# bark-simulator/planner-miqp

Measured on AMD Instinct MI355X. Metric: MIQP solves/sec to 1% gap, 2-agent x 20-step x 32-region, higher is better.
Workload: dtype f64

## Files before the change

planner_miqp_amd/csrc/kernels.hip:

```cpp
#include <hip/hip_runtime.h>

#include "host_inst.hpp"

#ifndef MIQP_RHO
#define MIQP_RHO 1.0e5
#endif

#ifndef MIQP_IPM_WPE
#define MIQP_IPM_WPE 3
#endif

#ifdef MIQP_ABLATE
#define MIQP_ABL (B.abl)
#else
#define MIQP_ABL 0
#endif
namespace miqp {

constexpr double RHO_EL = MIQP_RHO;
constexpr double FEAS_TOL = 1.0e-6;
constexpr double QP_TOL = 1.0e-6;
#ifndef MIQP_T0
#define MIQP_T0 1.0e-3
#endif
// ... 1936 lines not shown
    const double thr = B.far_cap > 0 && !B.inst_mode[inst] ? B.near_thr[inst] : 1e300;
    int nk = 0, nfar = 0, nnear = 0; double fmin_ = 1e300;
    for (int a = 0; a < nalt; ++a) {
      const double cb = objlb + clift[a];
      if (inc_now < 1e300 && (inc_now - cb) <= gapi * (1e-10 + fabs(inc_now))) { if (B.stats) atomicAdd(&B.stats[56], 1ull); continue; }
      int negm = 0;
      if (chosen.kind == 3 && ck[a] >= 0 && ck[a] < N && (B.seq_kinds & 0x10000) == 0) {
        negm = 1 << (int)comp[base + ck[a] * stride];
        for (int a2 = 1; a2 < a; ++a2) if (ck[a2] == ck[a]) negm |= 1 << ca[a2];
      }
      const bool tf = (cb - cst) > thr && B.batch_depth[node] != REPAIR_ROOT;
      k_ck[nk] = ck[a]; k_ca[nk] = ca[a]; k_neg[nk] = negm; k_ord[nk] = a; k_bnd[nk] = cb - cst;
      k_pos[nk] = tf ? (0x40000000 | nfar++) : nnear++;
      if (tf) fmin_ = fmin(fmin_, cb - cst);
      nk++;
    }
    int fbase = 0, obase = 0, ob2 = 0, extra2 = 0; bool okalloc = true;
    if (nnear > 0) {
      obase = atomicAdd(&B.open_count[inst], nnear);
      if (obase + nnear > B.open_cap) {
        for (int q = obase; q < obase + nnear && q < B.open_cap; ++q) { size_t oi = ((size_t)B.open_sel * B.n_slots + slot) * B.open_cap + q; B.open_bound[oi] = 1e300; B.open_node[oi] = -1; B.open_depth[oi] = 0; }
        if (B.far_cap > 0) { for (int q = 0; q < nk; ++q) if (!(k_pos[q] & 0x40000000)) { k_pos[q] = 0x40000000 | nfar++; fmin_ = fmin(fmin_, k_bnd[q]); } }
        else okalloc = false;
        nnear = 0; obase = 0;
      }
    }
    const int nnear_kept = nnear;
    if (nfar > 0) {
      fbase = atomicAdd(&B.far_count[inst], nfar);
      if (fbase + nfar <= B.far_cap) atomicMin(&B.far_minkey[inst], d2key(fmin_));
      else {
        for (int q = fbase; q < fbase + nfar && q < B.far_cap; ++q) { B.far_bound[(size_t)slot * B.far_cap + q] = 1e300; B.far_node[(size_t)slot * B.far_cap + q] = -1; }
        int extra = 0;
        for (int q = 0; q < nk; ++q) if (k_pos[q] & 0x40000000) k_pos[q] = 0x20000000 | extra++;
        nfar = 0;
        ob2 = atomicAdd(&B.open_count[inst], extra); extra2 = extra;
        if (ob2 + extra > B.open_cap) {
          okalloc = false;
          for (int q = ob2; q < ob2 + extra && q < B.open_cap; ++q) { size_t oi = ((size_t)B.open_sel * B.n_slots + slot) * B.open_cap + q; B.open_bound[oi] = 1e300; B.open_node[oi] = -1; B.open_depth[oi] = 0; }
        }
        sh_base[3] = ob2;
      }
    }
    if (okalloc && nk > 0) {
      unsigned int h = atomicAdd(B.free_head, (unsigned int)nk);
      if ((int)(*B.free_limit - h) >= nk) {
        for (int q = 0; q < nk; ++q) slots[q] = B.free_q[(h + q) % (unsigned int)B.pool_cap];
      } else {
        int nb = atomicAdd(B.pool_count, nk);
        if (nb + nk > B.pool_cap) okalloc = false;
        for (int q = 0; q < nk; ++q) slots[q] = nb + q;
      }
    }
    if (!okalloc) {
      atomicOr(&B.inst_flags[inst], 1);
      for (int q = fbase; q < fbase + nfar; ++q) { B.far_bound[(size_t)slot * B.far_cap + q] = 1e300; B.far_node[(size_t)slot * B.far_cap + q] = -1; }
      for (int q = obase; q < obase + nnear_kept && q < B.open_cap; ++q) { size_t oi = ((size_t)B.open_sel * B.n_slots + slot) * B.open_cap + q; B.open_bound[oi] = 1e300; B.open_node[oi] = -1; B.open_depth[oi] = 0; }
      for (int q = ob2; q < ob2 + extra2 && q < B.open_cap; ++q) { size_t oi = ((size_t)B.open_sel * B.n_slots + slot) * B.open_cap + q; B.open_bound[oi] = 1e300; B.open_node[oi] = -1; B.open_depth[oi] = 0; }
      nk = 0;
    }
    if (B.stats && nk > 0) { atomicAdd(&B.stats[43], 1ull); atomicAdd(&B.stats[44], (unsigned long long)nk); atomicAdd(&B.stats[48 + chosen.kind], 1ull); atomicAdd(&B.stats[52 + chosen.kind], (unsigned long long)nk); }
    sh_base[0] = fbase; sh_base[1] = obase; sh_base[2] = nk;
  }
  __syncthreads();
  PROF_T(te5);
  const int nk = sh_base[2];
  if (nk <= 0) { FREE_NODE(); return; }
  {
    for (int q = 0; q < nk; ++q) {
      signed char* dst = B.pool_fix + (size_t)slots[q] * Y.fixlen;
      const int kk = k_ck[q]; const signed char av = (signed char)k_ca[q];
      int negidx = -1; const int negm = k_neg[q];
      if (chosen.kind == 3 && kk >= 0 && kk < N && (B.seq_kinds & 0x10000) == 0) negidx = Y.f_c2n + (chosen.c * N + kk) * 4 + chosen.o;
      if (kk != -2) {
        for (int k8 = lane; k8 < Y.fixlen / 8; k8 += 64) ((unsigned long long*)cfix)[k8] = ((const unsigned long long*)fix)[k8];
        __syncthreads();
        for (int j = jlo + lane; j <= jhi; j += 64) { const int k = base + j * stride; if (fix[k] < 0) { if (j < kk) cfix[k] = comp[k]; else if (j == kk) cfix[k] = av; } }
        __syncthreads();
        if (lane == 0 && negidx >= 0) cfix[negidx] = (signed char)negm;
        __syncthreads();
        for (int k8 = lane; k8 < Y.fixlen / 8; k8 += 64) ((unsigned long long*)dst)[k8] = ((const unsigned long long*)cfix)[k8];
        __syncthreads();
      } else
      for (int k = lane; k < Y.fixlen; k += 64) {
        signed char v = fix[k];
        int rel = k - base;
        if (v < 0 && rel >= 0 && rel % stride == 0) {
          int j = rel / stride;
          if (j >= jlo && j <= jhi) { if (j < kk) v = comp[k]; else if (j == kk) v = av; }
        }
        if (k == negidx) v = (signed char)negm;
        if (kk == -2) {
          v = (fix[k] < 0 && k < Y.f_c2n) ? comp[k] : fix[k];
          if ((B.opt2 & 0x10000) && fix[k] < 0 && k >= Y.f_env && k < Y.f_c2c && (k - Y.f_env) % 5 != 0) v = fix[k];
          if (B.probe_margin > 0.0 && fix[k] < 0 && ploose[k]) v = fix[k];
        }
        dst[k] = v;
      }
      if (B.pool_origin && lane == 0) {
        int cls = k_ord[q] > 0 ? 1 : 0;
        if (chosen.kind == 0 && cls) { const int rq = (int)comp[base + chosen.i * stride] >> 2, cq = k_ca[q] >> 2; const int dq = T[Y.i_regj + chosen.c * P + cq] - T[Y.i_regj + chosen.c * P + rq]; const int ad = abs(dq) % Y.R;
          cls = (k_ca[q] & 3) == 3 ? 3 : ((ad == 1 || ad == Y.R - 1) ? 1 : 2); }
        B.pool_origin[slots[q]] = (signed char)(kk == -2 ? 15 : 4 * chosen.kind + cls);
      }
    }
    if (B.pool_big && lane < nk) B.pool_big[slots[lane]] = pumped ? (unsigned char)((((big_parent >> 4) + 1) << 4) | 1) : (unsigned char)(big_parent & ~12);
    if (B.pool_Z) {
      for (int q = 0; q < nk; ++q) { if (slots[q] >= B.z_cap) continue; double* zd = B.pool_Z + (size_t)slots[q] * N * NZ; for (int k = lane; k < N * NZ; k += 64) zd[k] = Z[k]; }
    }
    if (B.pool_A) {
      const bool as_node = B.batch_A && B.batch_large && B.batch_large[node] <= 1;
      const unsigned short av_ = as_node ? B.batch_A[(size_t)node * 64 + lane] : (unsigned short)0xFFFFu;
      for (int q = 0; q < nk; ++q) { if (slots[q] >= B.z_cap) continue; B.pool_A[(size_t)slots[q] * 64 + lane] = av_; }
      if (B.ring_M && lane < nk && slots[lane] < B.z_cap) B.pool_Mtag[slots[lane]] = as_node ? B.batch_Mtag[node] : 0ull;
    }
    if (lane < nk) {
      int pd = B.batch_depth[node] >> 6;
      int pref = k_ord[lane];
      if (B.opt2 & 2) {
        pref = 0;
        for (int q = 0; q < nk; ++q) if (k_bnd[q] < k_bnd[lane] || (k_bnd[q] == k_bnd[lane] && q < lane)) pref++;
      }
      const int dw = k_ck[lane] == -2 ? (((pd + 2) << 6) | 63) : (((pd + 1) << 6) | (62 - (pref < 62 ? pref : 62)));
      if (k_pos[lane] & 0x40000000) {
        size_t oi = (size_t)slot * B.far_cap + sh_base[0] + (k_pos[lane] & 0x3FFFFFFF);
        B.far_bound[oi] = k_bnd[lane]; B.far_node[oi] = slots[lane]; B.far_depth[oi] = dw;
      } else {
        const int np_ = (k_pos[lane] & 0x20000000) ? sh_base[3] + (k_pos[lane] & 0x1FFFFFFF) : sh_base[1] + k_pos[lane];
        size_t oi = ((size_t)B.open_sel * B.n_slots + slot) * B.open_cap + np_;
        B.open_bound[oi] = k_bnd[lane]; B.open_node[oi] = slots[lane]; B.open_depth[oi] = dw;
      }
    }
  }
  FREE_NODE();
#ifdef MIQP_PROFILE
  { PROF_T(te6);
    if (lane == 0) { atomicAdd(&B.prof[100], (unsigned long long)(te1 - te0)); atomicAdd(&B.prof[101], (unsigned long long)(te2 - te1)); atomicAdd(&B.prof[102], (unsigned long long)(te3 - te2));
                     atomicAdd(&B.prof[103], (unsigned long long)(te4 - te3)); atomicAdd(&B.prof[104], (unsigned long long)(te5 - te4)); atomicAdd(&B.prof[105], (unsigned long long)(te6 - te5)); atomicAdd(&B.prof[106], 1ull); } }
#endif
#undef FREE_NODE
}

constexpr int SEL_THREADS = 1024;
constexpr int SEL_LOWSHIFT = 24;

__device__ inline int wave_append(int* counter, bool pred) {
  const unsigned long long mk = __ballot(pred);
  const int lane = threadIdx.x & 63;
  int base = 0;
  if (lane == (int)(__ffsll((long long)mk) - 1)) base = atomicAdd(counter, __popcll(mk));
  base = __shfl(base, mk ? (int)(__ffsll((long long)mk) - 1) : 0);
  return base + __popcll(mk & ((1ull << lane) - 1ull));
}

__global__ void __launch_bounds__(SEL_THREADS) select_kernel(DevBuf B, int round) {
  const Layout& Y = B.Y;
  const int slot = blockIdx.x, tid = threadIdx.x;
#ifdef MIQP_PROFILE
  if (slot == 0 && tid == 0) {
    const unsigned long long a = B.prof[120], b = B.prof[121], c = B.prof[122];
    if (b != 0 && a != ~0ull && a != 0) { B.prof[123] += b - a; B.prof[124] += b - c; B.prof[125] += 1; }
    B.prof[120] = ~0ull; B.prof[121] = 0; B.prof[122] = ~0ull;
  }
#endif
  const int inst = B.slot_inst[slot];
  if (inst < 0 || B.inst_done[inst] || B.inst_kill[inst]) { if (tid == 0) B.slot_demand[slot] = 0; }
  if (inst < 0) return;
  const int cap = B.open_cap;
  __shared__ int sh_take, sh_base, sh_m, sh_keep, sh_pick, sh_ties, sh_w, sh_mv, sh_all, sh_elig;
  __shared__ double sh_inc;
  __shared__ unsigned int hist[256], dhist[256], sh_wsum[4];
  __shared__ int sh_bin;
  __shared__ int sh_dkeep, sh_tiecnt, sh_ndef;
  __shared__ unsigned long long sh_thr2;
  __shared__ unsigned long long sh_prefix, sh_thr, sh_fmin;
  __shared__ double red[SEL_THREADS];
  if (B.inst_done[inst]) return;
  const size_t src = ((size_t)B.open_sel * B.n_slots + slot) * cap, dst = ((size_t)(1 - B.open_sel) * B.n_slots + slot) * cap;
  unsigned long long* keys = B.open_key + (size_t)slot * cap;
  PROF_T(ts0);
  if (tid == 0) {
    unsigned long long key = B.inc_key[inst];
    sh_inc = inc_from_key(key);
    sh_take = -1;
    sh_thr = key != B.inc_seen[inst] ? key : ~0ull;
    sh_fmin = ~0ull;
    sh_m = 0; sh_keep = 0; sh_pick = 0; sh_ties = 0; sh_ndef = 0;
  }
  __syncthreads();
  if (sh_thr != ~0ull) {
    const unsigned long long key = sh_thr;
    const int pbc = B.prev_bc < B.batch_cap ? B.prev_bc : B.batch_cap;
    for (int k = tid; k < pbc; k += SEL_THREADS) if (B.batch_candkey[k] == key && B.batch_candinst[k] == inst) atomicMin(&sh_fmin, d2key(B.batch_obj[k]));
    __syncthreads();
    const unsigned long long bo = sh_fmin;
    if (tid == 0) sh_dkeep = 0x7FFFFFFF;
    __syncthreads();
    if (bo != ~0ull) for (int k = tid; k < pbc; k += SEL_THREADS) if (B.batch_candkey[k] == key && B.batch_candinst[k] == inst && d2key(B.batch_obj[k]) == bo) atomicMin(&sh_dkeep, k);
    __syncthreads();
    if (tid == 0 && sh_dkeep != 0x7FFFFFFF) { sh_take = sh_dkeep; B.inc_seen[inst] = key; }
  }
  __syncthreads();
  if (sh_take >= 0) {
    const int bslot = sh_take;
    const signed char* cf = B.batch_comp + (size_t)bslot * Y.fixlen; signed char* df = B.inc_fix + (size_t)inst * Y.fixlen;
    for (int k = tid; k < Y.fixlen; k += SEL_THREADS) df[k] = cf[k];
    const double* zs = B.batch_Z + (size_t)bslot * Y.N * Y.nz; double* zd = B.inc_Z + (size_t)inst * Y.N * Y.nz;
    for (int k = tid; k < Y.N * Y.nz; k += SEL_THREADS) zd[k] = zs[k];
    if (B.inc_A && B.batch_A && B.batch_Mtag) {
      if (tid < 64) B.inc_A[(size_t)inst * 64 + tid] = B.batch_A[(size_t)bslot * 64 + tid];
      if (tid == 0) B.inc_Mtag[inst] = B.batch_Mtag[bslot];
    }
    if (tid == 0) { B.inc_obj[inst] = B.batch_obj[bslot]; if (B.inst_lns) B.inst_lns[inst] |= 1; }
  }
  __syncthreads();
  if (B.inst_kill[inst]) {
    int nn = B.open_count[inst]; if (nn > cap) nn = cap;
    for (int k = tid; k < nn; k += SEL_THREADS) { const int nd = B.open_node[src + k]; if (nd >= 0) { unsigned int q_ = atomicAdd(B.free_tail, 1u); B.free_q[q_ % (unsigned int)B.pool_cap] = nd; } }
    int fn = B.far_cap > 0 ? B.far_count[inst] : 0; if (fn > B.far_cap) fn = B.far_cap;
    for (int k = tid; k < fn; k += SEL_THREADS) { const int nd = B.far_node[(size_t)slot * (size_t)B.far_cap + k]; if (nd >= 0) { unsigned int q_ = atomicAdd(B.free_tail, 1u); B.free_q[q_ % (unsigned int)B.pool_cap] = nd; } }
    __syncthreads();
    if (tid == 0) {
      B.open_count[inst] = 0; if (B.far_cap > 0) B.far_count[inst] = 0;
      atomicOr(&B.inst_flags[inst], 2); B.inst_done[inst] = 1; atomicSub(B.active_insts, 1);
    }
    return;
  }
  PROF_T(ts1);
  const double inc = fmin(sh_inc < 1e300 ? B.inc_obj[inst] : 1e300, B.inc_ext[inst]);
  const double cst = B.inst_const[inst];
  const double gap = B.inst_gap[inst];
  int n = B.open_count[inst]; if (n > cap) n = cap;
  auto prunable = [&](double b) { return inc < 1e300 && (inc - (b + cst)) <= gap * (1e-10 + fabs(inc)); };
  auto radix = [&](auto keyf, int cnt, int need) -> int {
    if (tid == 0) { sh_prefix = 0ull; sh_all = 0; }
    __syncthreads();
    for (int shift = 56; shift >= SEL_LOWSHIFT; shift -= 8) {
      if (tid < 256) hist[tid] = 0u;
      __syncthreads();
      const unsigned long long prefix = sh_prefix;
      const unsigned long long himask = shift == 56 ? 0ull : (~0ull << (shift + 8));
      for (int k = tid; k < cnt; k += SEL_THREADS) {
        unsigned long long key = keyf(k);
        if (key != ~0ull && (key & himask) == prefix) atomicAdd(&hist[(key >> shift) & 255ull], 1u);
      }
      __syncthreads();
      if (tid == 0) sh_bin = 256;
      unsigned int hv = 0, hx = 0;
      if (tid < 256) {
        hv = hist[tid]; hx = hv;
#pragma unroll
        for (int o = 1; o < 64; o <<= 1) { const unsigned int y = __shfl_up(hx, o); if ((tid & 63) >= o) hx += y; }
        if ((tid & 63) == 63) sh_wsum[tid >> 6] = hx;
      }
      __syncthreads();
      if (tid < 256) {
#pragma unroll
        for (int w = 0; w < 3; ++w) if (w < (tid >> 6)) hx += sh_wsum[w];
        if (hx >= (unsigned int)need) atomicMin(&sh_bin, tid);
        if (tid == 255) sh_wsum[3] = hx;
      }
      __syncthreads();
      {
        const int bin0 = sh_bin;
        if (tid == (bin0 < 256 ? bin0 : 255)) {
          const int bin = bin0 < 256 ? bin0 : 255;
          const unsigned int cum = bin0 < 256 ? hx - hv : sh_wsum[3];
          if (bin0 >= 256 && shift == 56) sh_all = 1;
          sh_prefix = prefix | ((unsigned long long)bin << shift);
          sh_pick = need - (int)cum;
          sh_tiecnt = (int)hv;
        }
      }
      __syncthreads();
      need = sh_pick;
      if (sh_all) break;
    }
    __syncthreads();
    return need;
  };
  const unsigned long long lowmask = (1ull << SEL_LOWSHIFT) - 1ull;
  int keep = cap / 4; { const int k2 = 2 * B.batch_cap > 65536 ? 2 * B.batch_cap : 65536; if (keep > k2) keep = k2; }
  const int spill_at = 2 * keep;
  const size_t fb = (size_t)slot * (size_t)B.far_cap;
  int fc = B.far_cap > 0 ? B.far_count[inst] : 0; if (fc > B.far_cap) fc = B.far_cap;
  const int dive_every = (B.seq_kinds >> 18) & 3;
  const bool periodic = dive_every == 0 ? (round & 3) == 3 : (dive_every == 1 ? false : (dive_every == 2 ? (round & 7) == 7 : (round & 1) == 1));
  bool pool_tight;
  { const int pc = *B.pool_count; const long long live = (long long)(pc < B.pool_cap ? pc : B.pool_cap) - (long long)(int)(*B.free_tail - *B.free_head);
    pool_tight = live > (long long)B.pool_cap / 10 * 9; }
  const bool lists_full = B.far_cap > 0 ? fc > B.far_cap / 4 * 3 : n > cap / 2;
  const bool dive = !(inc < 1e300) || periodic || lists_full || pool_tight;
  auto order_key = [&](double b, int dp) -> unsigned long long {
    const int dbias = (B.seq_kinds >> 24) & 3;
    const double bb = dbias ? b - (dbias == 1 ? 1e-4 : (dbias == 2 ? 1e-3 : 1e-2)) * fabs(b) * (double)(dp >> 6) : b;
    if (dive) { const unsigned long long kd = ((unsigned long long)(0xFFFF - (dp < 0xFFFF ? dp : 0xFFFF)) << 48) | (d2key(fmax(b, -1e300)) >> 16); return kd == ~0ull ? ~0ull - 1 : kd; }
    const double kv = fmax(bb, -1e300);
    const unsigned long long key = d2key(kv); return key == ~0ull ? ~0ull - 1 : key;
  };
  PROF_T(ts2);
  for (int k = tid; k < 256; k += SEL_THREADS) dhist[k] = 0u;
  __syncthreads();
  double lb = 1e300; int mloc = 0, ndef = 0;
  const bool big_round = B.probe_every <= 1 || (round % B.probe_every) == B.probe_every - 1;
  for (int k = tid; k < n; k += SEL_THREADS) {
    double b = B.open_bound[src + k]; int nd = B.open_node[src + k]; int dp = B.open_depth[src + k];
    unsigned long long key = ~0ull;
    if (nd < 0) { keys[k] = key; continue; }
    if (prunable(b)) {
      unsigned int q_ = atomicAdd(B.free_tail, 1u); B.free_q[q_ % (unsigned int)B.pool_cap] = nd;
    } else {
      lb = fmin(lb, b);
      key = order_key(b, dp);
      if (!big_round && is_probe_word(dp)) { key = ~0ull - 1; ndef++; }
      atomicAdd(&dhist[(dp >> 6) > 255 ? 255 : (dp >> 6)], 1u);
      mloc++;
    }
    keys[k] = key;
  }
  if (mloc) atomicAdd(&sh_m, mloc);
  if (ndef) atomicAdd(&sh_ndef, ndef);
  __syncthreads();
  int m = sh_m;
  PROF_T(ts3);
  if (fc > 0 && m < keep / 4 && cap - n >= 64) {
    auto fkey = [&](int k) -> unsigned long long {
      const double b = B.far_bound[fb + k];
      if (B.far_node[fb + k] < 0 || prunable(b)) return ~0ull;
      const unsigned long long key = d2key(b); return key == ~0ull ? ~0ull - 1 : key;
    };
    int stride = fc > 4 * keep ? (fc + keep - 1) / keep : 1;
    if (stride > 1 && (fc + stride - 1) / stride > cap - n) stride = (fc + (cap - n) - 1) / (cap - n);
    if (stride > 1) {
      const int ns = (fc + stride - 1) / stride;
      for (int j = tid; j < ns; j += SEL_THREADS) keys[n + j] = fkey(j * stride);
      __syncthreads();
      int need_s = (keep - m) / stride; if (need_s < 1) need_s = 1;
      radix([&](int k) { return keys[n + k]; }, ns, need_s);
    } else radix(fkey, fc, keep - m);
    const unsigned long long thr = sh_all ? ~0ull : sh_prefix;
    if (tid == 0) { sh_w = 0; sh_mv = 0; sh_fmin = ~0ull; }
    __syncthreads();
    int room = cap - n; if (room > keep - m) room = keep - m; if (room < 0) room = 0;
    constexpr int PER = 4;
    for (int c0 = 0; c0 < fc; c0 += SEL_THREADS * PER) {
      double eb[PER]; int en[PER], ed[PER], act[PER];
#pragma unroll
      for (int j = 0; j < PER; ++j) {
        const int k = c0 + j * SEL_THREADS + tid;
        act[j] = -1;
        if (k < fc) {
          eb[j] = B.far_bound[fb + k]; en[j] = B.far_node[fb + k]; ed[j] = B.far_depth[fb + k];
          if (en[j] < 0) act[j] = -1;
          else if (prunable(eb[j])) act[j] = 0;
          else { unsigned long long key = d2key(eb[j]); if (key == ~0ull) key = ~0ull - 1; act[j] = ((key & ~lowmask) <= thr) ? 2 : 1; }
        }
      }
      __syncthreads();
#pragma unroll
      for (int j = 0; j < PER; ++j) {
        if (act[j] == 0) { unsigned int q_ = atomicAdd(B.free_tail, 1u); B.free_q[q_ % (unsigned int)B.pool_cap] = en[j]; }
        int t = wave_append(&sh_mv, act[j] == 2);
        if (act[j] == 2) {
          if (t < room) {
            B.open_bound[src + n + t] = eb[j]; B.open_node[src + n + t] = en[j]; B.open_depth[src + n + t] = ed[j]; keys[n + t] = order_key(eb[j], ed[j]);
            lb = fmin(lb, eb[j]); atomicAdd(&dhist[(ed[j] >> 6) > 255 ? 255 : (ed[j] >> 6)], 1u);
          } else act[j] = 1;
        }
        int pos = wave_append(&sh_w, act[j] == 1);
        if (act[j] == 1) { B.far_bound[fb + pos] = eb[j]; B.far_node[fb + pos] = en[j]; B.far_depth[fb + pos] = ed[j]; atomicMin(&sh_fmin, d2key(eb[j])); }
      }
      __syncthreads();
    }
    const int moved = sh_mv < room ? sh_mv : room;
    n += moved; m += moved;
    fc = sh_w;
    __syncthreads();
    if (tid == 0) {
      B.far_count[inst] = fc; B.far_minkey[inst] = sh_fmin;
      B.near_thr[inst] = (fc > 0 && thr != ~0ull) ? key2d(thr | lowmask) : 1e300;
    }
  }
  PROF_T(ts4);
  lb = wave_min(lb);
  __syncthreads();
  if ((tid & 63) == 0) red[tid >> 6] = lb;
  __syncthreads();
#pragma unroll
  for (int w = 0; w < SEL_THREADS / 64; ++w) lb = fmin(lb, red[w]);
  if (fc > 0) lb = fmin(lb, key2d(B.far_minkey[inst]));
  const bool spill = B.far_cap > 0 && m > spill_at && fc < B.far_cap;
  unsigned long long thr_spill = ~0ull;
  if (spill) {
    radix([&](int k) { return keys[k]; }, n, keep);
    thr_spill = sh_all ? ~0ull : sh_prefix;
    if (tid == 0) { unsigned int cum = 0; int d = 255; for (; d >= 0; --d) { if (cum + dhist[d] > (unsigned int)(keep / 2)) break; cum += dhist[d]; } sh_dkeep = d + 1; }
    __syncthreads();
  }
  const int dkeep = sh_dkeep;
  PROF_T(ts5);
  if (tid == 0) sh_pick = 0;
  __syncthreads();
  const int act_now = *B.active_insts;
  const int focus_at = 16 << ((B.seq_kinds >> 29) & 3);
  const bool focus = act_now <= focus_at && inc < 1e300 && (B.seq_kinds & 0x8000000) == 0;
  if (focus) {
    const double gme = (inc - (lb + cst)) / (1e-10 + fabs(inc));
    int cntl = 0;
    for (int sj = tid; sj < B.n_slots; sj += SEL_THREADS) {
      const int j = B.slot_inst[sj];
      if (j < 0 || j == inst || B.inst_done[j]) continue;
      const double ij = B.inc_obj[j];
      const double gj = ij < 1e299 ? (ij - B.lower_bound[j]) / (1e-10 + fabs(ij)) : 1e300;
      if (gj < gme || (gj == gme && j < inst)) cntl++;
    }
    if (cntl) atomicAdd(&sh_pick, cntl);
  }
  __syncthreads();
  const int rank = sh_pick;
  __syncthreads();
  int m_elig = m - sh_ndef;
  if (!dive && inc < 1e300 && B.window_pct < 100 && m > 0) {
    const double top = inc - gap * (1e-10 + fabs(inc)) - cst;
    const double thrw = lb + 0.01 * (double)B.window_pct * fmax(0.0, top - lb);
    const unsigned long long kw = d2key(thrw);
    if (tid == 0) sh_elig = 0;
    __syncthreads();
    int ce = 0;
    for (int k = tid; k < n; k += SEL_THREADS) { const unsigned long long key = keys[k]; if (key != ~0ull && key <= kw) ce++; }
    if (ce) atomicAdd(&sh_elig, ce);
    __syncthreads();
    m_elig = sh_elig < 1 ? 1 : sh_elig;
    if (m_elig > m - sh_ndef) m_elig = m - sh_ndef;
  }
  if (tid == 0) {
    sh_pick = 0;
    int act = act_now; if (act < 1) act = 1;
    int w;
    if (B.seq_kinds & 0x40000000) {
      w = (focus && !(B.seq_kinds & 0x10000000)) ? (B.batch_cap >> (rank + 1 < 30 ? rank + 1 : 30)) : B.batch_cap / act;
      if (w < B.nodes_per_round) w = B.nodes_per_round;
    } else { w = B.slot_take[slot]; if (w < B.base_take && !(B.young_nodes > 0 && B.inst_nodes[inst] >= (long long)B.young_nodes)) w = B.base_take; }
    if (B.width_cap > 0 && w > B.width_cap) w = B.width_cap;
    if (!(inc < 1e300) && w > 512) w = 512;
    if (B.lns_narrow > 0 && B.inst_lns && (B.inst_lns[inst] & 1) && inc < 1e300 && B.inst_nodes[inst] >= (long long)B.lns_min_nodes && w > B.lns_narrow) w = B.lns_narrow;
    B.slot_demand[slot] = inc < 1e300 ? m_elig : (m < 512 ? m : 512);
    int take = m_elig < w ? m_elig : w;
    const int maxch = B.far_cap > 0 ? 8 : 64;
    int room = (cap - m) / maxch; if (room < 1) room = 1;
    if (B.far_cap > 0 && room < 1024) room = 1024;
    if (take > room) take = room;
    int base = take > 0 ? atomicAdd(B.batch_count, take) : 0;
    if (base + take > B.batch_cap) take = B.batch_cap > base ? B.batch_cap - base : 0;
    sh_take = take; sh_base = base;
    double lbt = ((n > 0 || fc > 0) && lb < 1e300 ? lb + cst : inc);
    if (inc < 1e300 && lbt > inc) lbt = inc;
    B.lower_bound[inst] = lbt;
    if (m == 0 && fc == 0) { B.inst_done[inst] = 1; atomicSub(B.active_insts, 1); }
    B.inst_mode[inst] = dive ? 1 : 0;
    sh_thr = ~0ull; sh_w = fc; sh_fmin = ~0ull;
  }
  __syncthreads();
  PROF_T(ts6);
  const int take = sh_take, base = sh_base;
  auto second_key = [&](unsigned long long key, int dp) -> unsigned long long { return (((key & lowmask) << 6) | (unsigned long long)(63 - (dp & 63))) << 34; };
  if (take > 0 && take < m) {
    int need = radix([&](int k) { return keys[k]; }, n, take);
    const unsigned long long thr1 = sh_prefix; const int tiecnt = sh_tiecnt;
    __syncthreads();
    unsigned long long thr2 = ~0ull;
    if (B.det_ties && need < tiecnt) {
      if (tiecnt <= SEL_THREADS) {
        unsigned long long* tie = (unsigned long long*)red;
        if (tid == 0) sh_elig = 0;
        __syncthreads();
        for (int k = tid; k < n; k += SEL_THREADS) {
          const unsigned long long key = keys[k];
          if (key != ~0ull && (key & ~lowmask) == thr1) { const int t = atomicAdd(&sh_elig, 1); if (t < SEL_THREADS) tie[t] = second_key(key, B.open_depth[src + k]); }
        }
        __syncthreads();
        const int tc = sh_elig < SEL_THREADS ? sh_elig : SEL_THREADS;
        if (tid < tc) {
          const unsigned long long v = tie[tid]; int lt = 0, le = 0;
          for (int j = 0; j < tc; ++j) { const unsigned long long u = tie[j]; lt += u < v ? 1 : 0; le += u <= v ? 1 : 0; }
          if (lt < need && need <= le) { sh_thr2 = v; sh_ties = need - lt; }
        }
        __syncthreads();
        thr2 = sh_thr2; need = sh_ties;
        __syncthreads();
      } else {
        need = radix([&](int k) -> unsigned long long { const unsigned long long key = keys[k]; if (key == ~0ull || (key & ~lowmask) != thr1) return ~0ull; return second_key(key, B.open_depth[src + k]); }, n, need);
        thr2 = sh_prefix;
        __syncthreads();
      }
    }
    if (tid == 0) { sh_thr = thr1; sh_thr2 = thr2; sh_ties = need; sh_pick = 0; }
    __syncthreads();
  } else if (tid == 0) { sh_thr = take >= m ? ~0ull : 0ull;    sh_thr2 = ~0ull; sh_ties = 0x7FFFFFFF; sh_pick = 0; }
  __syncthreads();
  PROF_T(ts7);
  const unsigned long long thr = sh_thr, thr2 = sh_thr2;
  for (int k0 = 0; k0 < n; k0 += SEL_THREADS) {
    const int k = k0 + tid;
    unsigned long long key = k < n ? keys[k] : ~0ull;
    const bool live = key != ~0ull;
    double b = 0.0; int nd = 0, dp = 0;
    bool pick = false;
    if (live) {
      b = B.open_bound[src + k]; nd = B.open_node[src + k]; dp = B.open_depth[src + k];
      if (take > 0) {
        const unsigned long long kh = key & (~0ull << SEL_LOWSHIFT);
        if (kh < thr) pick = true;
        else if (kh == thr) {
          const unsigned long long s2 = thr2 != ~0ull ? second_key(key, dp) : 0ull;
          if (thr2 != ~0ull && s2 < thr2) pick = true;
          else if (thr2 == ~0ull || s2 == thr2) { int t = atomicAdd(&sh_ties, -1); pick = t > 0; }
        }
      }
      if (pick) {
        int pos = atomicAdd(&sh_pick, 1);
        if (pos < take) { B.batch_node[base + pos] = nd; B.batch_inst[base + pos] = inst; B.batch_bound[base + pos] = b; B.batch_depth[base + pos] = dp;
                          if (B.batch_large) { const int lc_ = large_class(B, nd, dp, inc < 1e300); B.batch_large[base + pos] = (unsigned char)lc_;
                            if (lc_ && B.cls_list) { const int q_ = atomicAdd(&B.cls_count[lc_ - 1], 1); if (q_ < B.batch_cap) B.cls_list[(size_t)(lc_ - 1) * B.batch_cap + q_] = base + pos; } } }
        else pick = false;
      }
    }
    bool tofar = live && !pick && spill && (key & ~lowmask) > thr_spill && (dp >> 6) < dkeep;
    int fpos = wave_append(&sh_w, tofar);
    if (tofar) {
      if (fpos < B.far_cap) { B.far_bound[fb + fpos] = b; B.far_node[fb + fpos] = nd; B.far_depth[fb + fpos] = dp; atomicMin(&sh_fmin, d2key(b)); }
      else tofar = false;
    }
    const bool stay = live && !pick && !tofar;
    int pos = wave_append(&sh_keep, stay);
    if (stay) { B.open_bound[dst + pos] = b; B.open_node[dst + pos] = nd; B.open_depth[dst + pos] = dp; }
  }
  __syncthreads();
  if (tid == 0) {
    B.open_count[inst] = sh_keep;
    if (spill) {
      B.far_count[inst] = sh_w < B.far_cap ? sh_w : B.far_cap;
      if (sh_fmin != ~0ull) atomicMin(&B.far_minkey[inst], sh_fmin);
      B.near_thr[inst] = dive ? -1e300 : (thr_spill != ~0ull ? key2d(thr_spill | lowmask) : 1e300);
    }
  }
#ifdef MIQP_PROFILE
  { PROF_T(ts8);
    if (tid == 0) { const long long tt[9] = {ts0, ts1, ts2, ts3, ts4, ts5, ts6, ts7, ts8};
      for (int q = 0; q < 8; ++q) atomicAdd(&B.prof[110 + q], (unsigned long long)(tt[q + 1] - tt[q]));
      atomicAdd(&B.prof[118], 1ull); atomicAdd(&B.prof[119], (unsigned long long)n); } }
#endif
}

__global__ void admit_kernel(DevBuf B, const int* pairs, int n, int sel) {
  const int k = blockIdx.x * blockDim.x + threadIdx.x;
  if (k >= n) return;
  const int slot = pairs[2 * k], inst = pairs[2 * k + 1];
  const int old = B.slot_inst[slot];
  if (old >= 0) B.inst_slot[old] = -1;
  B.slot_inst[slot] = inst;
  if (inst < 0) return;
  B.inst_slot[inst] = slot;
  const int nr = B.root_cnt[inst];
  const size_t base = ((size_t)sel * B.n_slots + slot) * B.open_cap;
  for (int r = 0; r < nr; ++r) { B.open_bound[base + r] = -1e300; B.open_node[base + r] = B.root_node[(size_t)inst * B.root_stride + r]; B.open_depth[base + r] = B.root_depth[(size_t)inst * B.root_stride + r]; }
  B.open_count[inst] = nr;
  atomicAdd(B.active_insts, 1);
}

__global__ void __launch_bounds__(1024) share_kernel(DevBuf B) {
  __shared__ long long red[1024];
  __shared__ int sh_lo, sh_hi;
  const int tid = threadIdx.x, NSL = B.n_slots;
  const int WCAP = NSL == 1 ? (B.batch_cap > 8192 ? B.batch_cap : 8192) : 8192;
  auto bsum = [&](long long v) -> long long {
#pragma unroll
    for (int o = 32; o > 0; o >>= 1) v += __shfl_xor(v, o);
    __syncthreads();
    if ((tid & 63) == 0) red[tid >> 6] = v;
    __syncthreads();
    long long t = 0;
#pragma unroll
    for (int w = 0; w < 16; ++w) t += red[w];
    return t;
  };
  const long long target = (long long)B.batch_cap - (long long)B.batch_cap / 16;
  int base = B.base_take;
  if (B.floor_pct > 0) {
    if (tid == 0) { sh_lo = B.base_take; sh_hi = B.share_cap; }
    __syncthreads();
    const long long budget = target * B.floor_pct / 100;
    for (int itn = 0; itn < 12; ++itn) {
      const int lo = sh_lo, hi = sh_hi;
      if (lo >= hi) break;
      const int mid = lo + (hi - lo + 1) / 2;
      long long a = 0;
      for (int k = tid; k < NSL; k += 1024) { const int d = B.slot_demand[k]; a += d < mid ? d : mid; }
      const long long tot = bsum(a);
      if (tid == 0) { if (tot <= budget) sh_lo = mid; else sh_hi = mid - 1; }
      __syncthreads();
    }
    base = sh_lo;
    __syncthreads();
  }
  auto base_of = [&](int k) -> int {
    const int d = B.slot_demand[k], inst = B.slot_inst[k];
    if (B.young_nodes > 0 && inst >= 0 && B.inst_nodes[inst] >= (long long)B.young_nodes) return 0;
    return d < base ? d : base;
  };
  long long ab = 0;
  for (int k = tid; k < NSL; k += 1024) ab += base_of(k);
  const long long SB = bsum(ab);
  const long long rest = target - SB;
  const long long cap = B.share_cap;
  auto more_of = [&](int k) -> long long {
    const int d = B.slot_demand[k]; const long long c = d < cap ? d : cap;
    const int b = base_of(k);
    return c > b ? c - b : 0;
  };
  constexpr int SH_SLOTS = 2048;
  __shared__ int s_inst[SH_SLOTS]; __shared__ long long s_more[SH_SLOTS];
  const bool staged = NSL <= SH_SLOTS;
  if (staged) { for (int k = tid; k < NSL; k += 1024) { s_inst[k] = B.slot_inst[k]; s_more[k] = more_of(k); } }
  __syncthreads();
  long long at = 0;
  for (int k = tid; k < NSL; k += 1024) {
    const int inst = staged ? s_inst[k] : B.slot_inst[k];
    int take = base_of(k);
    const long long more = staged ? s_more[k] : more_of(k);
    if (inst >= 0 && more > 0 && rest > 0) {
      long long before = 0;
      if (staged) { for (int j = 0; j < NSL; ++j) { const int ij = s_inst[j]; if (ij >= 0 && ij < inst) before += s_more[j]; } }
      else { for (int j = 0; j < NSL; ++j) { const int ij = B.slot_inst[j]; if (ij >= 0 && ij < inst) before += more_of(j); } }
      long long ex = rest - before; if (ex > more) ex = more;
      if (ex > 0) take += (int)ex;
    }
    B.slot_take[k] = take; at += take;
  }
  const long long left = target - bsum(at);
  if (left <= 0) return;
  if (tid == 0) { sh_lo = 0; sh_hi = WCAP; }
  __syncthreads();
  for (int itn = 0; itn < 16; ++itn) {
    const int lo = sh_lo, hi = sh_hi;
    if (lo >= hi) break;
    const int mid = lo + (hi - lo + 1) / 2;
    long long a = 0;
    for (int k = tid; k < NSL; k += 1024) { long long r = (long long)B.slot_demand[k] - B.slot_take[k]; if (r > WCAP - B.slot_take[k]) r = WCAP - B.slot_take[k]; a += r < mid ? (r > 0 ? r : 0) : mid; }
    const long long tot = bsum(a);
    if (tid == 0) { if (tot <= left) sh_lo = mid; else sh_hi = mid - 1; }
    __syncthreads();
  }
  const int L = sh_lo;
  for (int k = tid; k < NSL; k += 1024) {
    long long r = (long long)B.slot_demand[k] - B.slot_take[k]; if (r > WCAP - B.slot_take[k]) r = WCAP - B.slot_take[k];
    if (r > 0) B.slot_take[k] += (int)(r < L ? r : L);
  }
}

constexpr int LNS_MAX = 512;
__global__ void __launch_bounds__(64) lns_kernel(DevBuf B) {
  const Layout& Y = B.Y;
  const int slot = blockIdx.x, lane = threadIdx.x;
  const int inst = B.slot_inst[slot];
  if (inst < 0) return;
  const int flags = B.inst_lns[inst];
  const bool want_skel = (B.lns_mode & 32) && !(flags & 2) && Y.NP > 0;
  if (!(flags & 1) && !want_skel) return;
  if (B.inst_nodes[inst] < (long long)B.lns_min_nodes) return;
  if ((flags & 1) && !want_skel && B.lns_step > 0.0) {
    const double io = B.inc_obj[inst] + B.inst_const[inst], last = B.inst_lns_obj[inst];
    if (last < 1e299 && io > last - B.lns_step * fabs(last)) return;
  }
  __shared__ int nb_c[LNS_MAX], nb_i[LNS_MAX], nb_n[LNS_MAX], nb_code[LNS_MAX];
  __shared__ int nb_c2[LNS_MAX], nb_n2[LNS_MAX], nb_code2[LNS_MAX];
  __shared__ int nb_rec[LNS_MAX];
  __shared__ int sh_n, sh_base, sh_rec, sh_skel;
  const int N = Y.N, C = Y.C;
  const signed char* inc = B.inc_fix + (size_t)inst * Y.fixlen;
  if (lane == 0) {
    int n = 0;
    auto push = [&](int first, int stride, int cnt, int val) { if (n < LNS_MAX) { nb_c[n] = first; nb_i[n] = stride; nb_n[n] = cnt; nb_code[n] = val; nb_n2[n] = 0; n++; } };
    const bool alive = !B.inst_done[inst] && !B.inst_kill[inst];
    sh_skel = 0;
    if (alive && want_skel) {
      sh_skel = 1;
      const int* T = B.inst_i + (size_t)inst * Y.istride;
      for (int p = 0; p < Y.NP; ++p) {
        const int first = Y.f_c2c + p * N * 4;
// ... 167 lines not shown
```

Before: 1061.

## Unroll select_kernel scans, track key range to skip radix passes, wave-reduce atomics

Several loops in the node-selection kernel are unrolled so each thread issues four independent loads before acting on them. The kernel also records the min and max of regular keys and starts the radix select at the first byte where they differ, skipping passes that cannot split the keys. Per-thread shared-memory atomics for counts and minimum keys are replaced by wave-level shuffle reductions followed by one atomic per wave. The far-list merge now prefetches the next chunk and drops a barrier per iteration. These add register pressure and code complexity in a 1024-thread block.

```diff
diff --git a/planner_miqp_amd/csrc/kernels.hip b/planner_miqp_amd/csrc/kernels.hip
--- a/planner_miqp_amd/csrc/kernels.hip
+++ b/planner_miqp_amd/csrc/kernels.hip
@@ -2112,6 +2112,31 @@
   base = __shfl(base, mk ? (int)(__ffsll((long long)mk) - 1) : 0);
   return base + __popcll(mk & ((1ull << lane) - 1ull));
 }
+__device__ inline unsigned long long wave_min_u64(unsigned long long v) {
+#pragma unroll
+  for (int o = 32; o > 0; o >>= 1) { const unsigned long long y = __shfl_xor(v, o); v = y < v ? y : v; }
+  return v;
+}
+__device__ inline unsigned long long wave_max_u64(unsigned long long v) {
+#pragma unroll
+  for (int o = 32; o > 0; o >>= 1) { const unsigned long long y = __shfl_xor(v, o); v = y > v ? y : v; }
+  return v;
+}
+__device__ inline int wave_sum_int(int v) {
+#pragma unroll
+  for (int o = 32; o > 0; o >>= 1) v += __shfl_xor(v, o);
+  return v;
+}
+constexpr int SEL_UNROLL = 4;
+__device__ inline int radix_first_shift(unsigned long long kmin, unsigned long long kmax, int lowshift, unsigned long long& prefix) {
+  prefix = 0ull;
+  if (kmin > kmax) return 56;
+  const unsigned long long diff = kmin ^ kmax;
+  int s = diff ? ((63 - __clzll((long long)diff)) & ~7) : lowshift;
+  if (s < lowshift) s = lowshift;
+  if (s < 56) prefix = kmin & (~0ull << (s + 8));
+  return s;
+}
 
 __global__ void __launch_bounds__(SEL_THREADS) select_kernel(DevBuf B, int round) {
   const Layout& Y = B.Y;
@@ -2134,6 +2159,8 @@
   __shared__ int sh_dkeep, sh_tiecnt, sh_ndef;
   __shared__ unsigned long long sh_thr2;
   __shared__ unsigned long long sh_prefix, sh_thr, sh_fmin;
+  __shared__ unsigned long long sh_kmin, sh_kmax;
+  __shared__ int sh_nreg;
   __shared__ double red[SEL_THREADS];
   if (B.inst_done[inst]) return;
   const size_t src = ((size_t)B.open_sel * B.n_slots + slot) * cap, dst = ((size_t)(1 - B.open_sel) * B.n_slots + slot) * cap;
@@ -2146,6 +2173,7 @@
     sh_thr = key != B.inc_seen[inst] ? key : ~0ull;
     sh_fmin = ~0ull;
     sh_m = 0; sh_keep = 0; sh_pick = 0; sh_ties = 0; sh_ndef = 0;
+    sh_kmin = ~0ull; sh_kmax = 0ull; sh_nreg = 0;
   }
   __syncthreads();
   if (sh_thr != ~0ull) {
@@ -2192,17 +2220,20 @@
   const double gap = B.inst_gap[inst];
   int n = B.open_count[inst]; if (n > cap) n = cap;
   auto prunable = [&](double b) { return inc < 1e300 && (inc - (b + cst)) <= gap * (1e-10 + fabs(inc)); };
-  auto radix = [&](auto keyf, int cnt, int need) -> int {
-    if (tid == 0) { sh_prefix = 0ull; sh_all = 0; }
+  auto radix = [&](auto keyf, int cnt, int need, int shift0, unsigned long long prefix0) -> int {
+    if (tid == 0) { sh_prefix = prefix0; sh_all = 0; }
     __syncthreads();
-    for (int shift = 56; shift >= SEL_LOWSHIFT; shift -= 8) {
+    for (int shift = shift0; shift >= SEL_LOWSHIFT; shift -= 8) {
       if (tid < 256) hist[tid] = 0u;
       __syncthreads();
       const unsigned long long prefix = sh_prefix;
       const unsigned long long himask = shift == 56 ? 0ull : (~0ull << (shift + 8));
-      for (int k = tid; k < cnt; k += SEL_THREADS) {
-        unsigned long long key = keyf(k);
-        if (key != ~0ull && (key & himask) == prefix) atomicAdd(&hist[(key >> shift) & 255ull], 1u);
+      for (int k0 = tid; k0 < cnt; k0 += SEL_THREADS * SEL_UNROLL) {
+        unsigned long long kv[SEL_UNROLL];
+#pragma unroll
+        for (int j = 0; j < SEL_UNROLL; ++j) { const int k = k0 + j * SEL_THREADS; kv[j] = k < cnt ? keyf(k) : ~0ull; }
+#pragma unroll
+        for (int j = 0; j < SEL_UNROLL; ++j) if (kv[j] != ~0ull && (kv[j] & himask) == prefix) atomicAdd(&hist[(kv[j] >> shift) & 255ull], 1u);
       }
       __syncthreads();
       if (tid == 0) sh_bin = 256;
@@ -2263,23 +2294,36 @@
   __syncthreads();
   double lb = 1e300; int mloc = 0, ndef = 0;
   const bool big_round = B.probe_every <= 1 || (round % B.probe_every) == B.probe_every - 1;
-  for (int k = tid; k < n; k += SEL_THREADS) {
-    double b = B.open_bound[src + k]; int nd = B.open_node[src + k]; int dp = B.open_depth[src + k];
-    unsigned long long key = ~0ull;
-    if (nd < 0) { keys[k] = key; continue; }
-    if (prunable(b)) {
-      unsigned int q_ = atomicAdd(B.free_tail, 1u); B.free_q[q_ % (unsigned int)B.pool_cap] = nd;
-    } else {
-      lb = fmin(lb, b);
-      key = order_key(b, dp);
-      if (!big_round && is_probe_word(dp)) { key = ~0ull - 1; ndef++; }
-      atomicAdd(&dhist[(dp >> 6) > 255 ? 255 : (dp >> 6)], 1u);
-      mloc++;
-    }
-    keys[k] = key;
-  }
-  if (mloc) atomicAdd(&sh_m, mloc);
-  if (ndef) atomicAdd(&sh_ndef, ndef);
+  unsigned long long kmin = ~0ull, kmax = 0ull; int nreg = 0;
+  for (int k0 = tid; k0 < n; k0 += SEL_THREADS * SEL_UNROLL) {
+    double eb[SEL_UNROLL]; int en[SEL_UNROLL], ed[SEL_UNROLL];
+#pragma unroll
+    for (int j = 0; j < SEL_UNROLL; ++j) {
+      const int k = k0 + j * SEL_THREADS;
+      if (k < n) { eb[j] = B.open_bound[src + k]; en[j] = B.open_node[src + k]; ed[j] = B.open_depth[src + k]; }
+    }
+#pragma unroll
+    for (int j = 0; j < SEL_UNROLL; ++j) {
+      const int k = k0 + j * SEL_THREADS;
+      if (k >= n) break;
+      const double b = eb[j]; const int nd = en[j], dp = ed[j];
+      unsigned long long key = ~0ull;
+      if (nd < 0) { keys[k] = key; continue; }
+      if (prunable(b)) {
+        unsigned int q_ = atomicAdd(B.free_tail, 1u); B.free_q[q_ % (unsigned int)B.pool_cap] = nd;
+      } else {
+        lb = fmin(lb, b);
+        key = order_key(b, dp);
+        if (!big_round && is_probe_word(dp)) { key = ~0ull - 1; ndef++; }
+        if (key < ~0ull - 1) { kmin = key < kmin ? key : kmin; kmax = key > kmax ? key : kmax; nreg++; }
+        atomicAdd(&dhist[(dp >> 6) > 255 ? 255 : (dp >> 6)], 1u);
+        mloc++;
+      }
+      keys[k] = key;
+    }
+  }
+  mloc = wave_sum_int(mloc); ndef = wave_sum_int(ndef);
+  if ((tid & 63) == 0) { if (mloc) atomicAdd(&sh_m, mloc); if (ndef) atomicAdd(&sh_ndef, ndef); }
   __syncthreads();
   int m = sh_m;
   PROF_T(ts3);
@@ -2293,45 +2337,63 @@
     if (stride > 1 && (fc + stride - 1) / stride > cap - n) stride = (fc + (cap - n) - 1) / (cap - n);
     if (stride > 1) {
       const int ns = (fc + stride - 1) / stride;
-      for (int j = tid; j < ns; j += SEL_THREADS) keys[n + j] = fkey(j * stride);
+      for (int j0 = tid; j0 < ns; j0 += SEL_THREADS * SEL_UNROLL) {
+        unsigned long long kv[SEL_UNROLL];
+#pragma unroll
+        for (int u = 0; u < SEL_UNROLL; ++u) { const int j = j0 + u * SEL_THREADS; kv[u] = j < ns ? fkey(j * stride) : ~0ull; }
+#pragma unroll
+        for (int u = 0; u < SEL_UNROLL; ++u) { const int j = j0 + u * SEL_THREADS; if (j < ns) keys[n + j] = kv[u]; }
+      }
       __syncthreads();
       int need_s = (keep - m) / stride; if (need_s < 1) need_s = 1;
-      radix([&](int k) { return keys[n + k]; }, ns, need_s);
-    } else radix(fkey, fc, keep - m);
+      radix([&](int k) { return keys[n + k]; }, ns, need_s, 56, 0ull);
+    } else radix(fkey, fc, keep - m, 56, 0ull);
     const unsigned long long thr = sh_all ? ~0ull : sh_prefix;
     if (tid == 0) { sh_w = 0; sh_mv = 0; sh_fmin = ~0ull; }
     __syncthreads();
     int room = cap - n; if (room > keep - m) room = keep - m; if (room < 0) room = 0;
     constexpr int PER = 4;
+    double nb[PER]; int nn_[PER], ndp[PER];
+    unsigned long long fmin_l = ~0ull;
+    auto fload = [&](int c0) {
+#pragma unroll
+      for (int j = 0; j < PER; ++j) {
+        const int k = c0 + j * SEL_THREADS + tid;
+        nb[j] = 0.0; nn_[j] = -1; ndp[j] = 0;
+        if (k < fc) { ndp[j] = B.far_depth[fb + k]; nb[j] = B.far_bound[fb + k]; nn_[j] = B.far_node[fb + k]; }
+      }
+    };
+    fload(0);
     for (int c0 = 0; c0 < fc; c0 += SEL_THREADS * PER) {
       double eb[PER]; int en[PER], ed[PER], act[PER];
 #pragma unroll
       for (int j = 0; j < PER; ++j) {
-        const int k = c0 + j * SEL_THREADS + tid;
-        act[j] = -1;
-        if (k < fc) {
-          eb[j] = B.far_bound[fb + k]; en[j] = B.far_node[fb + k]; ed[j] = B.far_depth[fb + k];
-          if (en[j] < 0) act[j] = -1;
-          else if (prunable(eb[j])) act[j] = 0;
-          else { unsigned long long key = d2key(eb[j]); if (key == ~0ull) key = ~0ull - 1; act[j] = ((key & ~lowmask) <= thr) ? 2 : 1; }
-        }
+        eb[j] = nb[j]; en[j] = nn_[j]; ed[j] = ndp[j];
+        if (en[j] < 0) act[j] = -1;
+        else if (prunable(eb[j])) act[j] = 0;
+        else { unsigned long long key = d2key(eb[j]); if (key == ~0ull) key = ~0ull - 1; act[j] = ((key & ~lowmask) <= thr) ? 2 : 1; }
       }
       __syncthreads();
+      if (c0 + SEL_THREADS * PER < fc) fload(c0 + SEL_THREADS * PER);
 #pragma unroll
       for (int j = 0; j < PER; ++j) {
         if (act[j] == 0) { unsigned int q_ = atomicAdd(B.free_tail, 1u); B.free_q[q_ % (unsigned int)B.pool_cap] = en[j]; }
         int t = wave_append(&sh_mv, act[j] == 2);
         if (act[j] == 2) {
           if (t < room) {
-            B.open_bound[src + n + t] = eb[j]; B.open_node[src + n + t] = en[j]; B.open_depth[src + n + t] = ed[j]; keys[n + t] = order_key(eb[j], ed[j]);
+            const unsigned long long key = order_key(eb[j], ed[j]);
+            B.open_bound[src + n + t] = eb[j]; B.open_node[src + n + t] = en[j]; B.open_depth[src + n + t] = ed[j]; keys[n + t] = key;
+            if (key < ~0ull - 1) { kmin = key < kmin ? key : kmin; kmax = key > kmax ? key : kmax; nreg++; }
             lb = fmin(lb, eb[j]); atomicAdd(&dhist[(ed[j] >> 6) > 255 ? 255 : (ed[j] >> 6)], 1u);
           } else act[j] = 1;
         }
         int pos = wave_append(&sh_w, act[j] == 1);
-        if (act[j] == 1) { B.far_bound[fb + pos] = eb[j]; B.far_node[fb + pos] = en[j]; B.far_depth[fb + pos] = ed[j]; atomicMin(&sh_fmin, d2key(eb[j])); }
-      }
-      __syncthreads();
-    }
+        if (act[j] == 1) { B.far_bound[fb + pos] = eb[j]; B.far_node[fb + pos] = en[j]; B.far_depth[fb + pos] = ed[j]; const unsigned long long fk = d2key(eb[j]); fmin_l = fk < fmin_l ? fk : fmin_l; }
+      }
+    }
+    fmin_l = wave_min_u64(fmin_l);
+    if ((tid & 63) == 0 && fmin_l != ~0ull) atomicMin(&sh_fmin, fmin_l);
+    __syncthreads();
     const int moved = sh_mv < room ? sh_mv : room;
     n += moved; m += moved;
     fc = sh_w;
@@ -2343,16 +2405,22 @@
   }
   PROF_T(ts4);
   lb = wave_min(lb);
-  __syncthreads();
-  if ((tid & 63) == 0) red[tid >> 6] = lb;
+  kmin = wave_min_u64(kmin); kmax = wave_max_u64(kmax);
+  __syncthreads();
+  if ((tid & 63) == 0) { red[tid >> 6] = lb; if (kmin <= kmax) { atomicMin(&sh_kmin, kmin); atomicMax(&sh_kmax, kmax); } }
+  nreg = wave_sum_int(nreg);
+  if ((tid & 63) == 0 && nreg) atomicAdd(&sh_nreg, nreg);
   __syncthreads();
 #pragma unroll
   for (int w = 0; w < SEL_THREADS / 64; ++w) lb = fmin(lb, red[w]);
   if (fc > 0) lb = fmin(lb, key2d(B.far_minkey[inst]));
   const bool spill = B.far_cap > 0 && m > spill_at && fc < B.far_cap;
   unsigned long long thr_spill = ~0ull;
+  unsigned long long kpre = 0ull;
+  const int kshift = radix_first_shift(sh_kmin, sh_kmax, SEL_LOWSHIFT, kpre);
+  const int nreg_all = sh_nreg;
   if (spill) {
-    radix([&](int k) { return keys[k]; }, n, keep);
+    radix([&](int k) { return keys[k]; }, n, keep, keep <= nreg_all ? kshift : 56, keep <= nreg_all ? kpre : 0ull);
     thr_spill = sh_all ? ~0ull : sh_prefix;
     if (tid == 0) { unsigned int cum = 0; int d = 255; for (; d >= 0; --d) { if (cum + dhist[d] > (unsigned int)(keep / 2)) break; cum += dhist[d]; } sh_dkeep = d + 1; }
     __syncthreads();
@@ -2387,8 +2455,12 @@
     if (tid == 0) sh_elig = 0;
     __syncthreads();
     int ce = 0;
-    for (int k = tid; k < n; k += SEL_THREADS) { const unsigned long long key = keys[k]; if (key != ~0ull && key <= kw) ce++; }
-    if (ce) atomicAdd(&sh_elig, ce);
+    for (int k0 = tid; k0 < n; k0 += SEL_THREADS * SEL_UNROLL) {
+#pragma unroll
+      for (int j = 0; j < SEL_UNROLL; ++j) { const int k = k0 + j * SEL_THREADS; const unsigned long long key = k < n ? keys[k] : ~0ull; if (key != ~0ull && key <= kw) ce++; }
+    }
+    ce = wave_sum_int(ce);
+    if ((tid & 63) == 0 && ce) atomicAdd(&sh_elig, ce);
     __syncthreads();
     m_elig = sh_elig < 1 ? 1 : sh_elig;
     if (m_elig > m - sh_ndef) m_elig = m - sh_ndef;
@@ -2425,7 +2497,7 @@
   const int take = sh_take, base = sh_base;
   auto second_key = [&](unsigned long long key, int dp) -> unsigned long long { return (((key & lowmask) << 6) | (unsigned long long)(63 - (dp & 63))) << 34; };
   if (take > 0 && take < m) {
-    int need = radix([&](int k) { return keys[k]; }, n, take);
+    int need = radix([&](int k) { return keys[k]; }, n, take, take <= nreg_all ? kshift : 56, take <= nreg_all ? kpre : 0ull);
     const unsigned long long thr1 = sh_prefix; const int tiecnt = sh_tiecnt;
     __syncthreads();
     unsigned long long thr2 = ~0ull;
@@ -2434,9 +2506,15 @@
         unsigned long long* tie = (unsigned long long*)red;
         if (tid == 0) sh_elig = 0;
         __syncthreads();
-        for (int k = tid; k < n; k += SEL_THREADS) {
-          const unsigned long long key = keys[k];
-          if (key != ~0ull && (key & ~lowmask) == thr1) { const int t = atomicAdd(&sh_elig, 1); if (t < SEL_THREADS) tie[t] = second_key(key, B.open_depth[src + k]); }
+        for (int k0 = tid; k0 < n; k0 += SEL_THREADS * SEL_UNROLL) {
+          unsigned long long kv[SEL_UNROLL];
+#pragma unroll
+          for (int j = 0; j < SEL_UNROLL; ++j) { const int k = k0 + j * SEL_THREADS; kv[j] = k < n ? keys[k] : ~0ull; }
+#pragma unroll
+          for (int j = 0; j < SEL_UNROLL; ++j) {
+            const unsigned long long key = kv[j];
+            if (key != ~0ull && (key & ~lowmask) == thr1) { const int t = atomicAdd(&sh_elig, 1); if (t < SEL_THREADS) tie[t] = second_key(key, B.open_depth[src + k0 + j * SEL_THREADS]); }
+          }
         }
         __syncthreads();
         const int tc = sh_elig < SEL_THREADS ? sh_elig : SEL_THREADS;
@@ -2449,7 +2527,7 @@
         thr2 = sh_thr2; need = sh_ties;
         __syncthreads();
       } else {
-        need = radix([&](int k) -> unsigned long long { const unsigned long long key = keys[k]; if (key == ~0ull || (key & ~lowmask) != thr1) return ~0ull; return second_key(key, B.open_depth[src + k]); }, n, need);
+        need = radix([&](int k) -> unsigned long long { const unsigned long long key = keys[k]; if (key == ~0ull || (key & ~lowmask) != thr1) return ~0ull; return second_key(key, B.open_depth[src + k]); }, n, need, 56, 0ull);
         thr2 = sh_prefix;
         __syncthreads();
       }
@@ -2460,41 +2538,55 @@
   __syncthreads();
   PROF_T(ts7);
   const unsigned long long thr = sh_thr, thr2 = sh_thr2;
-  for (int k0 = 0; k0 < n; k0 += SEL_THREADS) {
-    const int k = k0 + tid;
-    unsigned long long key = k < n ? keys[k] : ~0ull;
-    const bool live = key != ~0ull;
-    double b = 0.0; int nd = 0, dp = 0;
-    bool pick = false;
-    if (live) {
-      b = B.open_bound[src + k]; nd = B.open_node[src + k]; dp = B.open_depth[src + k];
-      if (take > 0) {
-        const unsigned long long kh = key & (~0ull << SEL_LOWSHIFT);
-        if (kh < thr) pick = true;
-        else if (kh == thr) {
-          const unsigned long long s2 = thr2 != ~0ull ? second_key(key, dp) : 0ull;
-          if (thr2 != ~0ull && s2 < thr2) pick = true;
-          else if (thr2 == ~0ull || s2 == thr2) { int t = atomicAdd(&sh_ties, -1); pick = t > 0; }
-        }
-      }
-      if (pick) {
-        int pos = atomicAdd(&sh_pick, 1);
-        if (pos < take) { B.batch_node[base + pos] = nd; B.batch_inst[base + pos] = inst; B.batch_bound[base + pos] = b; B.batch_depth[base + pos] = dp;
-                          if (B.batch_large) { const int lc_ = large_class(B, nd, dp, inc < 1e300); B.batch_large[base + pos] = (unsigned char)lc_;
-                            if (lc_ && B.cls_list) { const int q_ = atomicAdd(&B.cls_count[lc_ - 1], 1); if (q_ < B.batch_cap) B.cls_list[(size_t)(lc_ - 1) * B.batch_cap + q_] = base + pos; } } }
-        else pick = false;
-      }
-    }
-    bool tofar = live && !pick && spill && (key & ~lowmask) > thr_spill && (dp >> 6) < dkeep;
-    int fpos = wave_append(&sh_w, tofar);
-    if (tofar) {
-      if (fpos < B.far_cap) { B.far_bound[fb + fpos] = b; B.far_node[fb + fpos] = nd; B.far_depth[fb + fpos] = dp; atomicMin(&sh_fmin, d2key(b)); }
-      else tofar = false;
-    }
-    const bool stay = live && !pick && !tofar;
-    int pos = wave_append(&sh_keep, stay);
-    if (stay) { B.open_bound[dst + pos] = b; B.open_node[dst + pos] = nd; B.open_depth[dst + pos] = dp; }
-  }
+  unsigned long long fmin_l = ~0ull;
+  for (int kk = 0; kk < n; kk += SEL_THREADS * SEL_UNROLL) {
+    unsigned long long ek[SEL_UNROLL]; double eb[SEL_UNROLL]; int en[SEL_UNROLL], ed[SEL_UNROLL];
+#pragma unroll
+    for (int j = 0; j < SEL_UNROLL; ++j) { const int k = kk + j * SEL_THREADS + tid; ek[j] = k < n ? keys[k] : ~0ull; }
+#pragma unroll
+    for (int j = 0; j < SEL_UNROLL; ++j) {
+      const int k = kk + j * SEL_THREADS + tid;
+      eb[j] = 0.0; en[j] = 0; ed[j] = 0;
+      if (ek[j] != ~0ull) { eb[j] = B.open_bound[src + k]; en[j] = B.open_node[src + k]; ed[j] = B.open_depth[src + k]; }
+    }
+#pragma unroll
+    for (int j = 0; j < SEL_UNROLL; ++j) {
+      if (kk + j * SEL_THREADS >= n) break;
+      const unsigned long long key = ek[j];
+      const bool live = key != ~0ull;
+      const double b = eb[j]; const int nd = en[j], dp = ed[j];
+      bool pick = false;
+      if (live) {
+        if (take > 0) {
+          const unsigned long long kh = key & (~0ull << SEL_LOWSHIFT);
+          if (kh < thr) pick = true;
+          else if (kh == thr) {
+            const unsigned long long s2 = thr2 != ~0ull ? second_key(key, dp) : 0ull;
+            if (thr2 != ~0ull && s2 < thr2) pick = true;
+            else if (thr2 == ~0ull || s2 == thr2) { int t = atomicAdd(&sh_ties, -1); pick = t > 0; }
+          }
+        }
+        if (pick) {
+          int pos = atomicAdd(&sh_pick, 1);
+          if (pos < take) { B.batch_node[base + pos] = nd; B.batch_inst[base + pos] = inst; B.batch_bound[base + pos] = b; B.batch_depth[base + pos] = dp;
+                            if (B.batch_large) { const int lc_ = large_class(B, nd, dp, inc < 1e300); B.batch_large[base + pos] = (unsigned char)lc_;
+                              if (lc_ && B.cls_list) { const int q_ = atomicAdd(&B.cls_count[lc_ - 1], 1); if (q_ < B.batch_cap) B.cls_list[(size_t)(lc_ - 1) * B.batch_cap + q_] = base + pos; } } }
+          else pick = false;
+        }
+      }
+      bool tofar = live && !pick && spill && (key & ~lowmask) > thr_spill && (dp >> 6) < dkeep;
+      int fpos = wave_append(&sh_w, tofar);
+      if (tofar) {
+        if (fpos < B.far_cap) { B.far_bound[fb + fpos] = b; B.far_node[fb + fpos] = nd; B.far_depth[fb + fpos] = dp; const unsigned long long fk = d2key(b); fmin_l = fk < fmin_l ? fk : fmin_l; }
+        else tofar = false;
+      }
+      const bool stay = live && !pick && !tofar;
+      int pos = wave_append(&sh_keep, stay);
+      if (stay) { B.open_bound[dst + pos] = b; B.open_node[dst + pos] = nd; B.open_depth[dst + pos] = dp; }
+    }
+  }
+  fmin_l = wave_min_u64(fmin_l);
+  if ((tid & 63) == 0 && fmin_l != ~0ull) atomicMin(&sh_fmin, fmin_l);
   __syncthreads();
   if (tid == 0) {
     B.open_count[inst] = sh_keep;
```

Result: no change. 1058 (-0.3%).
